# hashicorp/consul

Hardware: NVIDIA B200
Metric: million node-ticks/sec (higher is better)
Workload: dtype u32

## Files before the change

__graft_entry__.py:

```python
from __future__ import annotations

import os
import subprocess
import sys

ROOT = os.path.dirname(os.path.abspath(__file__))
CSRC = os.path.join(ROOT, "consul_b200", "csrc")
LIBGSIM = os.path.join(ROOT, "consul_b200", "libgsim.so")
LIBORACLE = os.path.join(ROOT, "oracle", "liboracle.so")
LIBHOSTEMU = os.path.join(ROOT, "tests", "hostemu", "libgsim_hostemu.so")
FACADE_DEMO = os.path.join(ROOT, "tests", "hostemu", "serf_facade_check")

NVCC_FLAGS = ["-gencode", "arch=compute_100a,code=sm_100a", "-lineinfo", "-O3", "-std=c++17", "-fmad=false",
              "-Xcompiler", "-fPIC", "-Xcompiler", "-ffp-contract=off", "-Xcompiler", "-pthread", "-shared"]


def _newer(target: str, sources) -> bool:
    if not os.path.exists(target):
        return False
    t = os.path.getmtime(target)
    return all(os.path.getmtime(s) <= t for s in sources)


def _run(cmd):
    print("+", " ".join(cmd), flush=True)
    subprocess.run(cmd, check=True, cwd=ROOT)


def _sources(*dirs_and_ext):
    out = []
    for d, exts in dirs_and_ext:
        for f in sorted(os.listdir(d)):
            if f.endswith(exts):
                out.append(os.path.join(d, f))
    return out


def build_oracle(force: bool = False) -> None:
    hdr = _sources((os.path.join(ROOT, "include"), (".h",)))
    osrc = [os.path.join(ROOT, "oracle", "oracle.cpp")]
    if force or not _newer(LIBORACLE, osrc + hdr):
        _run(["g++", "-O3", "-mavx2", "-ffp-contract=off", "-std=c++17", "-fopenmp", "-fPIC", "-shared", "-o",
              LIBORACLE] + osrc)


def build(force: bool = False) -> None:
    hdr = _sources((CSRC, (".h",)), (os.path.join(ROOT, "include"), (".h", ".hpp")))
    srcs = [os.path.join(CSRC, "gs_cuda.cu"), os.path.join(CSRC, "gs_vmm.cu"), os.path.join(CSRC, "gs_api.cpp")]
    if force or not _newer(LIBGSIM, srcs + hdr):
        nvcc = os.environ.get("NVCC", "nvcc")
        _run([nvcc] + NVCC_FLAGS + ["-o", LIBGSIM] + srcs)
    build_oracle(force)
    hsrc = [os.path.join(CSRC, "gs_api.cpp"), os.path.join(ROOT, "tests", "hostemu", "hostemu_backend.cpp")]
    if force or not _newer(LIBHOSTEMU, hsrc + hdr):
        _run(["g++", "-O2", "-ffp-contract=off", "-std=c++17", "-pthread", "-fPIC", "-shared",
              "-DGS_MAKE_BACKEND=gs_make_hostemu_backend", "-o", LIBHOSTEMU] + hsrc)
    sys.path.insert(0, ROOT)
    import consul_b200


def smoke() -> None:
    sys.path.insert(0, ROOT)
    sys.path.insert(0, os.path.join(ROOT, "tests"))
    if not (os.path.exists(LIBGSIM) and os.path.exists(LIBORACLE)):
        build()
    from consul_b200 import Pool, lan_config, PRED_ALL_RUMORS_CONVERGED
    from oracle_binding import OraclePool

    n = 4096
    cfg = lan_config(capacity=n + 1, n_initial=n, seed=0x5EED0001)
    gpu = Pool(cfg)
    ora = OraclePool(cfg)
    for p in (gpu, ora):
        x = p.member_add()
        assert p.join(x, [0]) == 1
    tg = gpu.run_until(PRED_ALL_RUMORS_CONVERGED, 0, 400, 1)
    to = ora.run_until(PRED_ALL_RUMORS_CONVERGED, 0, 400, 1)
    gpu.step(64)
    ora.step(64)
    hg, ho = gpu.state_hash(), ora.state_hash()
    assert tg == to, (tg, to)
    assert hg == ho, (hg, ho)
    assert gpu.launch_count() > 0
    print(f"smoke ok: n={n + 1} converged at tick {tg}, state hash {hg[0]:016x} == oracle, "
          f"{gpu.launch_count()} kernel launches")


if __name__ == "__main__":
    build(force="--force" in sys.argv)
    if "--smoke" in sys.argv:
        smoke()
```

consul_b200/csrc/gs_api.cpp:

```cpp
#include <math.h>
#include <stdio.h>
#include <stdlib.h>
#include <string.h>

#include <algorithm>
#include <mutex>
#include <string>
#include <type_traits>
#include <atomic>
#include <condition_variable>
#include <functional>
#include <thread>
#include <vector>

#include "../../include/gsim.h"
#include "gs_backend.h"
#include "gs_wire.h"
#include "gs_coord.h"

#ifndef GS_MAKE_BACKEND
#define GS_MAKE_BACKEND gs_make_cuda_backend
#endif
GsBackend* GS_MAKE_BACKEND(int device, char* err, size_t err_cap);

// ... 608 lines not shown
    okk = okk && acol(&tx16, GS_MAX_RUMORS / 2);
    d.tx = reinterpret_cast<uint8_t*>(tx16);
  }
  if (cfg->flags & GSIM_FLAG_COORDINATES) {
    if (sharded) {
      g_create_err = "network coordinates are not supported on sharded pools yet";
      fprintf(stderr, "libgsim: %s\n", g_create_err.c_str());
      gsim_pool_destroy(p);
      return GSIM_ERR_INVALID;
    }
    okk = okk && alloc_col(p, &d.coord, cap * 2 * GS_COORD_WORDS) && alloc_col(p, &d.ctag, cap * 2) &&
          alloc_col(p, &d.adj, cap * GS_ADJ_WINDOW) && alloc_col(p, &d.adj_idx, cap);
  }
  if (cfg->flags & GSIM_FLAG_PUSH_PULL)
    okk = okk && acol(&d.ppreq, 2 * GS_PPK) && acol(&d.pp_clk, 4);
  uint32_t evcap = cfg->event_log_capacity ? cfg->event_log_capacity : 65536u;
  if (!sharded) {
    okk = okk && alloc_col(p, &d.stats, (size_t)GSIM_STAT_COUNT);
    okk = okk && alloc_col(p, &d.heard_cnt, (size_t)32) && alloc_col(p, &d.conv_tick, (size_t)32);
    okk = okk && alloc_col(p, &d.view_cnt, (size_t)4);
    okk = okk && alloc_col(p, &d.crashed_alive, (size_t)1) && alloc_col(p, &d.crashed_dead_tick, (size_t)1);
    okk = okk && alloc_col(p, &d.evlog, (size_t)evcap) && alloc_col(p, &d.evlog_cursor, (size_t)2);
    okk = okk && alloc_col(p, &d.tick_base, (size_t)1);
    okk = okk && alloc_col(p, &d.done_ctr, (size_t)1);
    okk = okk && alloc_col(p, &d.qstate[0], (size_t)GS_Q_WORDS);
    okk = okk && alloc_col(p, &p->g_dev, (size_t)1);
  } else if (okk) {
    p->pages = reinterpret_cast<uint8_t*>(be->shard_alloc(GS_PAGE_BYTES, 1));
    okk = p->pages != nullptr && be->shard_commit(&p->shard_fds, &p->n_shard_fds);
    if (okk) {
      uint8_t* page0 = p->pages;
      uint8_t* mine = p->pages + (size_t)p->rank * GS_PAGE_BYTES;
      d.stats = reinterpret_cast<unsigned long long*>(mine + GS_PG_STATS);
      d.heard_cnt = reinterpret_cast<uint32_t*>(page0 + GS_PG_HEARD_CNT);
      d.conv_tick = reinterpret_cast<uint32_t*>(page0 + GS_PG_CONV_TICK);
      d.view_cnt = reinterpret_cast<uint32_t*>(page0 + GS_PG_VIEW_CNT);
      d.crashed_alive = reinterpret_cast<uint32_t*>(page0 + GS_PG_CRASHED_ALIVE);
      d.crashed_dead_tick = reinterpret_cast<uint32_t*>(page0 + GS_PG_CRASHED_DEAD_TICK);
      d.evlog_cursor = reinterpret_cast<uint32_t*>(page0 + GS_PG_EVLOG_CURSOR);
      d.evlog = reinterpret_cast<GsEventRec*>(page0 + GS_PG_EVLOG);
      const uint32_t room = (GS_PAGE_BYTES - GS_PG_EVLOG) / (uint32_t)sizeof(GsEventRec);
      if (evcap > room) evcap = room;
      d.tick_base = reinterpret_cast<uint32_t*>(mine + GS_PG_TICK_BASE);
      p->g_dev = reinterpret_cast<GsGlobals*>(mine + GS_PG_GLOBALS);
      for (uint32_t r = 0; r < GS_MAX_WORLD; ++r)
        p->xb.flags[r] = reinterpret_cast<uint32_t*>(p->pages + (size_t)(r < p->world ? r : 0) * GS_PAGE_BYTES + GS_PG_XBAR_FLAGS);
      for (uint32_t r = 0; r < GS_MAX_WORLD; ++r)
        d.tick_flags[r] = reinterpret_cast<uint32_t*>(p->pages + (size_t)(r < p->world ? r : 0) * GS_PAGE_BYTES + GS_PG_TICK_FLAGS);
      d.done_ctr = reinterpret_cast<uint32_t*>(mine + GS_PG_DONE_CTR);
      for (uint32_t r = 0; r < p->world; ++r)
        d.qstate[r] = reinterpret_cast<uint32_t*>(p->pages + (size_t)r * GS_PAGE_BYTES + GS_PG_QSTATE);
      p->xb.epoch = reinterpret_cast<uint32_t*>(mine + GS_PG_XBAR_EPOCH);
      p->xb.rank = p->rank;
      p->xb.world = p->world;
      okk = be->fill8(mine, 0, GS_PAGE_BYTES) && be->sync();
    }
  }
  if (!okk) {
    g_create_err = be->last_error();
    fprintf(stderr, "libgsim: allocation failed: %s\n", be->last_error());
    gsim_pool_destroy(p);
    return GSIM_ERR_NOMEM;
  }

  g.n = cfg->n_initial;
  p->n_established = cfg->n_initial;
  g.cap = (uint32_t)cap;
  g.up_count = cfg->n_initial;
  g.P = (uint32_t)(cfg->probe_interval_ns / tick);
  g.T = (uint32_t)(cfg->probe_timeout_ns / tick);
  g.GI = (uint32_t)(cfg->gossip_interval_ns / tick);
  g.gossip_nodes = cfg->gossip_nodes;
  g.indirect_checks = cfg->indirect_checks;
  g.awareness_max = cfg->awareness_max_multiplier;
  g.gtd_ticks = ceil_ticks(cfg->gossip_to_the_dead_ns, tick);
  g.udp_avail = cfg->udp_buffer_size > 2 ? cfg->udp_buffer_size - 2 : 0;
  g.disable_tcp = cfg->disable_tcp_pings;
  g.loss_thr = (uint32_t)(((uint64_t)cfg->packet_loss_ppm << 32) / 1000000ull);
  if (cfg->packet_loss_ppm >= 1000000u) g.loss_thr = 0xFFFFFFFFu;
  g.event_buffer = cfg->event_buffer;
  g.seed_lo = (uint32_t)cfg->seed;
  g.seed_hi = (uint32_t)(cfg->seed >> 32);
  g.flags = cfg->flags;
  g.evlog_cap = evcap;
  g.world = cfg->world_size;
  g.rank = cfg->rank;
  g.phase_group = phase_group;
  g.phase_gate = (phase_group % GS_TILE == 0) ? 1u : 0u;
  g.phase_shift = 0;
  while (g.phase_gate && (GS_TILE << g.phase_shift) < phase_group) g.phase_shift++;
  {
    const uint32_t rot = gs_phase_rot(g.seed_lo, g.seed_hi);
    g.rot_p = rot % g.P;
    g.rot_g = (rot >> 16) % g.GI;
  }
  g.rows_per_rank = (uint32_t)p->rows_per_rank;
  g.tick_seconds = (double)tick / 1.0e9;
  g.coord_base_rtt_s = 0.0005;
  recompute_tables(p);
  if (!sharded && init_device_state(p) != GSIM_OK) {
    g_create_err = be->last_error();
    fprintf(stderr, "libgsim: pool init failed: %s\n", be->last_error());
    gsim_pool_destroy(p);
    return GSIM_ERR_CUDA;
  }
  *out = p;
  return GSIM_OK;
}

extern "C" int gsim_shard_export_fds(gsim_pool* p, int* fds, size_t cap, size_t* n) {
  if (!p || !n || !p->sharded) return GSIM_ERR_INVALID;
  *n = p->n_shard_fds;
  if (fds) {
    if (cap < p->n_shard_fds) return GSIM_ERR_INVALID;
    memcpy(fds, p->shard_fds, p->n_shard_fds * sizeof(int));
  }
  return GSIM_OK;
}

extern "C" int gsim_shard_attach(gsim_pool* p, uint32_t peer_rank, const int* fds, size_t n) {
  if (!p || !p->sharded || p->ready || !fds) return GSIM_ERR_INVALID;
  std::lock_guard<std::mutex> lk(p->mu);
  if (!p->be->shard_attach(peer_rank, fds, n)) return fail(p, GSIM_ERR_CUDA, "shard_attach");
  p->attached += 1;
  return GSIM_OK;
}

extern "C" int gsim_shard_ready(gsim_pool* p) {
  if (!p) return GSIM_ERR_INVALID;
  if (!p->sharded) return GSIM_OK;
  std::lock_guard<std::mutex> lk(p->mu);
  if (p->ready) return GSIM_OK;
  if (p->attached != p->world) return fail(p, GSIM_ERR_STATE, "not every peer rank has been attached");
  if (!p->be->xbar_host(p->xb)) return fail(p, GSIM_ERR_CUDA, "barrier");
  int rc = controller_call(p, nullptr, 0, [&]() -> int { return init_device_state(p); });
  if (rc) return fail(p, rc, "init");
  p->ready = true;
  return GSIM_OK;
}

extern "C" void gsim_pool_destroy(gsim_pool* p) {
  if (!p) return;
  if (p->be) {
    p->be->sync();
    if (p->stage) p->be->host_free(p->stage);
    delete p->workers;
    p->workers = nullptr;
    for (void* q : p->allocs) p->be->release(q);
    delete p->be;
  }
  delete p;
}

static void shard_rows(const gsim_pool* p, uint32_t* first, uint32_t* count) {
  const uint32_t n = p->g.n;
  *first = 0;
  *count = n;
  if (p->sharded) {
    const uint64_t f = (uint64_t)p->rank * p->rows_per_rank;
    *first = f < n ? (uint32_t)f : n;
    *count = *first + p->rows_per_rank < n ? (uint32_t)p->rows_per_rank : n - *first;
  }
}

static int collective_recount(gsim_pool* p) {
  if (!p->sharded || !p->ready) return GSIM_OK;
// ... 1584 lines not shown
```

consul_b200/csrc/gs_cuda.cu:

```cuda
#include <cuda_runtime.h>
#include <stdio.h>
#include <stdlib.h>
#include <string.h>

#include <map>

#include "gs_aux.h"
#include "gs_backend.h"
#include "gs_vmm.h"

#define GS_BLOCK 256
#define GS_GRAPH_TICKS 64
#define GS_WIN_GRAPH 8

namespace {

template <bool COORDS>
struct DevSinkT {
  static constexpr bool kCoords = COORDS;
  uint32_t* s_stat;
  uint32_t* s_heard;
  uint32_t* s_q;
  __device__ __forceinline__ void activity() { s_q[0] = 1u; }
  __device__ __forceinline__ void horizon(uint32_t h) { atomicMin(&s_q[1], h); }
// ... 17 lines not shown
      e.reserved = 0u;
      d.evlog[pos] = e;
    } else {
      atomicAdd_system(&d.evlog_cursor[1], 1u);
    }
  }
};
typedef DevSinkT<false> DevSink;

#ifndef GS_MIN_BLOCKS
#define GS_MIN_BLOCKS 4
#endif
#define GS_WARPS (GS_BLOCK / 32)
#define GS_ROUND 4

__device__ __forceinline__ uint32_t gs_smem_addr(const void* p) { return (uint32_t)__cvta_generic_to_shared(p); }
__device__ __forceinline__ void gs_mbar_init(uint64_t* bar, uint32_t arrivals) {
  asm volatile("mbarrier.init.shared::cta.b64 [%0], %1;" ::"r"(gs_smem_addr(bar)), "r"(arrivals) : "memory");
}
__device__ __forceinline__ void gs_mbar_expect_tx(uint64_t* bar, uint32_t bytes) {
  asm volatile("mbarrier.arrive.expect_tx.shared::cta.b64 _, [%0], %1;" ::"r"(gs_smem_addr(bar)), "r"(bytes) : "memory");
}
__device__ __forceinline__ void gs_bulk_g2s(void* smem_dst, const void* gsrc, uint32_t bytes, uint64_t* bar) {
  asm volatile("cp.async.bulk.shared::cluster.global.mbarrier::complete_tx::bytes [%0], [%1], %2, [%3];" ::"r"(
                   gs_smem_addr(smem_dst)),
               "l"(gsrc), "r"(bytes), "r"(gs_smem_addr(bar))
               : "memory");
}
__device__ __forceinline__ bool gs_mbar_wait(uint64_t* bar, uint32_t parity) {
  for (uint32_t spin = 0; spin < (1u << 24); ++spin) {
    uint32_t done;
    asm volatile(
        "{\n\t.reg .pred p;\n\t"
        "mbarrier.try_wait.parity.shared::cta.b64 p, [%1], %2;\n\t"
        "selp.u32 %0, 1, 0, p;\n\t}"
        : "=r"(done)
        : "r"(gs_smem_addr(bar)), "r"(parity)
        : "memory");
    if (done) return true;
  }
  return false;
}

__device__ __forceinline__ void gs_ranks_wait(const GsDev& d, const GsGlobals& g, uint32_t t) {
  if (threadIdx.x < g.world) {
    uint32_t v;
    do {
      asm volatile("ld.acquire.sys.global.u32 %0, [%1];" : "=r"(v) : "l"(d.tick_flags[g.rank] + threadIdx.x) : "memory");
    } while ((int32_t)(v - t) < 0);
  }
  __syncthreads();
}
__device__ __forceinline__ void gs_ranks_release(const GsDev& d, const GsGlobals& g, uint32_t t_done) {
  __syncthreads();
  if (threadIdx.x == 0u) {
    __threadfence_system();
    const uint32_t arrived = atomicAdd(d.done_ctr, 1u);
    if (arrived == gridDim.x - 1u) {
      __threadfence_system();
      *d.done_ctr = 0u;
      __threadfence_system();
      for (uint32_t r = 0; r < g.world; ++r)
        asm volatile("st.release.sys.global.u32 [%0], %1;" ::"l"(d.tick_flags[r] + g.rank), "r"(t_done) : "memory");
    }
  }
}

__device__ __forceinline__ void gs_q_publish(const GsDev& d, const GsGlobals& g, const uint32_t* s_q, uint32_t t) {
  if (s_q[0] != 0u) {
    if (g.world <= 1u) atomicMax(d.qstate[0] + GS_Q_LAST_ACTIVE, t + 1u);
    else for (uint32_t r = 0; r < g.world; ++r) atomicMax_system(d.qstate[r] + GS_Q_LAST_ACTIVE, t + 1u);
  }
  if (s_q[1] != GS_NEVER) {
    if (g.world <= 1u) atomicMin(d.qstate[0] + GS_Q_HORIZON, s_q[1]);
    else for (uint32_t r = 0; r < g.world; ++r) atomicMin_system(d.qstate[r] + GS_Q_HORIZON, s_q[1]);
  }
}

template <bool COORDS>
__device__ __noinline__ void gs_row_step_call(const GsDev* dp, const GsGlobals* gp, uint32_t i, uint32_t t,
                                              uint32_t inb, uint32_t* s_stat, uint32_t* s_heard, uint32_t* s_q) {
  DevSinkT<COORDS> sink{s_stat, s_heard, s_q};
  gs_row_step(*dp, *gp, i, t, t % gp->GI, inb, sink);
}

template <bool COORDS>
__global__ void __launch_bounds__(GS_BLOCK, GS_MIN_BLOCKS)
    gs_tick_kernel(const __grid_constant__ GsDev d, const GsGlobals* __restrict__ gp, uint32_t k_off) {
  __shared__ uint32_t s_stat[GS_NSTAT * 32];
  __shared__ uint32_t s_heard[32 * 32];
  __shared__ __align__(128) uint32_t s_inb[GS_WARPS][GS_ROUND][GS_TILE];
  __shared__ __align__(128) uint32_t s_due[GS_WARPS][GS_ROUND][GS_TILE];
  __shared__ __align__(8) uint64_t s_bar[GS_WARPS];
  __shared__ uint32_t s_q[2];
  __shared__ uint32_t s_work[GS_WARPS * GS_ROUND * 4];
  __shared__ uint32_t s_wn[2], s_wtake[2];
  const uint32_t tid = threadIdx.x;
  for (uint32_t x = tid; x < GS_NSTAT * 32u; x += GS_BLOCK) s_stat[x] = 0u;
  for (uint32_t x = tid; x < 32u * 32u; x += GS_BLOCK) s_heard[x] = 0u;
  if (tid == 64u) s_q[0] = 0u;
  if (tid == 65u) s_q[1] = GS_NEVER;
  if (tid >= 66u && tid < 68u) s_wn[tid - 66u] = 0u;
  if (tid >= 68u && tid < 70u) s_wtake[tid - 68u] = 0u;
  if (tid >= 96u && tid < 96u + GS_WARPS) gs_mbar_init(&s_bar[tid - 96u], 1u);
  asm volatile("fence.mbarrier_init.release.cluster;" ::: "memory");
  asm volatile("griddepcontrol.launch_dependents;" ::: "memory");
  asm volatile("griddepcontrol.wait;" ::: "memory");
  __syncthreads();
  const GsGlobals& g = *gp;
  const uint32_t t = *d.tick_base + k_off;
  if (g.world > 1u) gs_ranks_wait(d, g, t);
  const uint32_t cur = t & 1u, P = g.P, pslot = t % P, gslot = t % g.GI;
  const uint32_t pslot_t = (t + P - g.T % P) % P;
  const uint32_t lane = tid & 31u, wib = tid >> 5;
  uint32_t tile_lo = 0, tile_hi = (g.n + GS_TILE - 1u) / GS_TILE;
  if (g.world > 1u) {
    const uint32_t per = g.rows_per_rank / GS_TILE;
    tile_lo = g.rank * per < tile_hi ? g.rank * per : tile_hi;
    tile_hi = tile_lo + per < tile_hi ? tile_lo + per : tile_hi;
  }
  const uint32_t n_warps = gridDim.x * GS_WARPS, n_tiles = tile_hi - tile_lo;
  const uint32_t wid = blockIdx.x * GS_WARPS + wib;
  const uint32_t t_begin = tile_lo + (uint32_t)(((uint64_t)wid * n_tiles) / n_warps);
  const uint32_t t_end = tile_lo + (uint32_t)(((uint64_t)(wid + 1u) * n_tiles) / n_warps);
  const uint32_t* __restrict__ inbox_cur = d.inbox[t & g.ring_mask];
  const bool gated = g.phase_gate != 0u;
  const uint32_t shift = g.phase_shift;
  DevSinkT<COORDS> sink{s_stat, s_heard, s_q};

  const uint32_t max_run = (n_tiles + n_warps - 1u) / n_warps, n_rounds = (max_run + GS_ROUND - 1u) / GS_ROUND;
  bool did_work = false;
  const bool sys_scan = g.world > 1u && (g.flags & 4u);
  auto bring = [&](uint32_t r) {
    const uint32_t b0 = t_begin + r * GS_ROUND < t_end ? t_begin + r * GS_ROUND : t_end;
    const uint32_t b1 = b0 + GS_ROUND < t_end ? b0 + GS_ROUND : t_end;
    const uint32_t tiles = b1 - b0;
    if (!tiles) return;
    uint32_t gate_mask = 0;
    for (uint32_t x = 0; x < tiles; ++x) {
      bool gate = true;
      if (gated) {
        const uint32_t pp = gs_probe_phase(g.rot_p, (b0 + x) >> shift, P);
        gate = pp == pslot || pp == pslot_t;
      }
      gate_mask |= gate ? 1u << x : 0u;
    }
    const size_t off0 = (size_t)b0 * GS_TILE;
    if (sys_scan) {
      for (uint32_t x = 0; x < tiles; ++x) {
        uint4 v;
        asm volatile("ld.relaxed.sys.global.v4.u32 {%0,%1,%2,%3}, [%4];"
                     : "=r"(v.x), "=r"(v.y), "=r"(v.z), "=r"(v.w) : "l"(inbox_cur + off0 + x * GS_TILE + lane * 4u) : "memory");
        *reinterpret_cast<uint4*>(&s_inb[wib][x][lane * 4u]) = v;
        const uint4 dv = (gate_mask >> x) & 1u ? *reinterpret_cast<const uint4*>(d.due + off0 + x * GS_TILE + lane * 4u)
                                               : make_uint4(GS_NEVER, GS_NEVER, GS_NEVER, GS_NEVER);
        *reinterpret_cast<uint4*>(&s_due[wib][x][lane * 4u]) = dv;
      }
      __syncwarp();
      return;
    }
    for (uint32_t x = 0; x < tiles; ++x)
      if (!((gate_mask >> x) & 1u))
        *reinterpret_cast<uint4*>(&s_due[wib][x][lane * 4u]) = make_uint4(GS_NEVER, GS_NEVER, GS_NEVER, GS_NEVER);
    __syncwarp();
    if (lane == 0u) {
      asm volatile("fence.proxy.async.shared::cta;" ::: "memory");
// ... 4 lines not shown
    }
  };
  bring(0u);
  for (uint32_t round = 0; round < n_rounds; ++round) {
  const uint32_t par = round & 1u;
  const uint32_t r_begin = t_begin + round * GS_ROUND < t_end ? t_begin + round * GS_ROUND : t_end;
  const uint32_t r_end = r_begin + GS_ROUND < t_end ? r_begin + GS_ROUND : t_end;
  if (r_end > r_begin && !sys_scan && !gs_mbar_wait(&s_bar[wib], round & 1u)) {
    if (lane == 0u) atomicExch(d.qstate[g.rank] + GS_Q_VIOLATION, t + 1u);
  }
  for (uint32_t tile = r_begin; tile < r_end; ++tile) {
    const uint32_t st = tile - r_begin;
    const uint4 i4 = *reinterpret_cast<const uint4*>(&s_inb[wib][st][lane * 4u]);
    const uint4 d4 = *reinterpret_cast<const uint4*>(&s_due[wib][st][lane * 4u]);
    bool mine = (i4.x | i4.y | i4.z | i4.w) != 0u || d4.x == t || d4.y == t || d4.z == t || d4.w == t;
    bool pp_tile = false;
    if (g.pp_interval != 0u) {
      if (gated) {
        pp_tile = gs_pp_due(g.pp_interval, g.rot_pp, tile >> shift, t);
      } else {
#pragma unroll
        for (uint32_t u = 0; u < 4u; ++u)
          pp_tile |= gs_pp_due(g.pp_interval, g.rot_pp, (tile * GS_TILE + lane * 4u + u) / g.phase_group, t);
      }
      mine |= pp_tile;
    }
    if (__any_sync(0xFFFFFFFFu, mine)) {
      did_work = true;
      __syncwarp();
      const uint32_t base = tile * GS_TILE + lane;
      bool act[4], cand[4];
      bool any_cand = false;
#pragma unroll
      for (int u = 0; u < 4; ++u) {
        const uint32_t w = s_inb[wib][st][u * 32 + lane];
        const bool due_now = s_due[wib][st][u * 32 + lane] == t;
        act[u] = w != 0u || due_now ||
                 (g.pp_interval != 0u && gs_pp_due(g.pp_interval, g.rot_pp, (base + 32u * u) / g.phase_group, t));
        cand[u] = w == 0u && due_now;
        any_cand |= cand[u];
      }
      if (__any_sync(0xFFFFFFFFu, any_cand)) {
        GsFastProbe f[4];
#pragma unroll
        for (int u = 0; u < 4; ++u)
          if (cand[u]) gs_fast_load(d, cur, base + 32u * u, f[u]);
#pragma unroll
        for (int u = 0; u < 4; ++u)
          if (cand[u]) cand[u] = gs_fast_target(d, g, cur, base + 32u * u, f[u]);
        uint32_t n_probe = 0, n_ack = 0;
#pragma unroll
        for (int u = 0; u < 4; ++u) {
          bool acked = false;
          const bool done = cand[u] && gs_fast_finish(d, g, sink, base + 32u * u, t, f[u], &acked);
          if (done) act[u] = false;
          n_probe += __popc(__ballot_sync(0xFFFFFFFFu, done));
          n_ack += __popc(__ballot_sync(0xFFFFFFFFu, done && acked));
        }
        if (lane == 0u && n_probe) {
          atomicAdd(&s_stat[GS_ST_PROBES * 32], n_probe);
          atomicAdd(&s_stat[GS_ST_ACTIVE_ROWS * 32], n_probe);
          if (n_ack) atomicAdd(&s_stat[GS_ST_ACKS * 32], n_ack);
        }
      }
#pragma unroll
      for (int u = 0; u < 4; ++u) {
        if (__any_sync(0xFFFFFFFFu, act[u]) && lane == 0u) s_work[atomicAdd(&s_wn[par], 1u)] = tile * 4u + (uint32_t)u;
      }
    }
  }
  __syncwarp();
  if (round + 1u < n_rounds) bring(round + 1u);
  __syncthreads();
  if (tid == 0u) s_wn[par ^ 1u] = s_wtake[par ^ 1u] = 0u;
  const uint32_t n_work = s_wn[par];
  for (;;) {
    uint32_t idx = 0;
    if (lane == 0u) idx = atomicAdd(&s_wtake[par], 1u);
    idx = __shfl_sync(0xFFFFFFFFu, idx, 0);
    if (idx >= n_work) break;
    did_work = true;
    const uint32_t i = s_work[idx] * 32u + lane;
    const uint32_t w = __ldcg(inbox_cur + i);
    const bool a = w != 0u || __ldcg(d.due + i) == t ||
                   (g.pp_interval != 0u && gs_pp_due(g.pp_interval, g.rot_pp, i / g.phase_group, t));
    if (a) gs_row_step_call<COORDS>(&d, gp, i, t, w, s_stat, s_heard, s_q);
  }
  __syncthreads();
  }
  if (g.world > 1u && did_work && !(g.flags & 8u)) __threadfence_system();
  __syncthreads();
  if (tid < GS_NSTAT) {
    uint32_t v = 0;
    for (uint32_t x = 0; x < 32u; ++x) v += s_stat[tid * 32u + ((x + tid) & 31u)];
    if (v) atomicAdd(&d.stats[tid], (unsigned long long)v);
  } else if (tid >= 32u && tid < 32u + GS_MAX_RUMORS) {
    uint32_t r = tid - 32u, c = 0;
    for (uint32_t x = 0; x < 32u; ++x) c += s_heard[r * 32u + ((x + r) & 31u)];
    if (c) {
      uint32_t old = atomicAdd_system(&d.heard_cnt[r], c);
      if (old + c == g.up_count) d.conv_tick[r] = t;
    }
  }
  if (tid == 0u) gs_q_publish(d, g, s_q, t);
  if (g.world > 1u) gs_ranks_release(d, g, t + 1u);
}

template <bool COORDS>
__device__ __noinline__ void gs_window_generic(const GsDev* dp, const GsGlobals* gp, uint32_t gb, uint32_t g_end,
                                               uint32_t tf00, uint32_t tf01, uint32_t tf02, uint32_t tf03,
                                               uint32_t tx00, uint32_t tx01, uint32_t tx02, uint32_t tx03,
                                               uint32_t t0, uint32_t w1, uint32_t* s_stat, uint32_t* s_heard,
                                               uint32_t* s_q, uint32_t* counts) {
  const GsDev& d = *dp;
  const GsGlobals& g = *gp;
  const GsHot h = gs_hot(g);
  const uint32_t P = h.P, T = h.T, lane = threadIdx.x & 31u;
  const uint32_t tf0[4] = {tf00, tf01, tf02, tf03}, tx0[4] = {tx00, tx01, tx02, tx03};
  const bool fast_ok = h.loss_thr == 0u && h.graph_n == 0u && d.coord == nullptr && h.pp_interval == 0u;
  DevSinkT<COORDS> sink{s_stat, s_heard, s_q};
  uint32_t n_probe = 0, n_ack = 0;
  bool did_work = false;
  (void)did_work;
#pragma unroll 1
    for (uint32_t s0 = t0; s0 < w1; s0 += P) {
    const uint32_t off = s0 - t0;
    uint32_t tf[4], tx[4], due[4];
    bool cand[4], slow[4];
    bool any_slow = false;
#pragma unroll
    for (int u = 0; u < 4; ++u) {
      if (gb + u < g_end) {
        tf[u] = tf0[u] + off;
        tx[u] = tx0[u] + off;
        due[u] = __ldcg(d.due + (gb + u) * 32u + lane);
      } else {
        tf[u] = tx[u] = GS_NEVER;
        due[u] = GS_NEVER - 1u;
      }
      cand[u] = fast_ok && due[u] == tf[u] && tf[u] < w1;
      slow[u] = (due[u] == tf[u] && tf[u] < w1 && !fast_ok) || (due[u] == tx[u] && tx[u] < w1);
    }
    GsFastProbe f[4];
#pragma unroll
    for (int u = 0; u < 4; ++u)
      if (cand[u]) gs_fast_load(d, tf[u] & 1u, (gb + u) * 32u + lane, f[u]);
#pragma unroll
    for (int u = 0; u < 4; ++u)
      if (cand[u]) {
        const bool okk = gs_fast_target(d, h, tf[u] & 1u, (gb + u) * 32u + lane, f[u]);
        if (!okk) { cand[u] = false; slow[u] = true; }
      }
#pragma unroll
    for (int u = 0; u < 4; ++u) {
      bool acked = false, done = false;
      if (cand[u]) {
        done = gs_fast_finish(d, h, sink, (gb + u) * 32u + lane, tf[u], f[u], &acked);
        if (!done) slow[u] = true;
        else if (!acked && tf[u] + T < w1) slow[u] = true;
      }
      n_probe += done ? 1u : 0u;
      n_ack += done && acked ? 1u : 0u;
      any_slow |= slow[u];
    }
    if (__any_sync(0xFFFFFFFFu, any_slow)) {
      did_work = true;
#pragma unroll 1
      for (int u = 0; u < 4; ++u) {
        const bool sl = u == 0 ? slow[0] : u == 1 ? slow[1] : u == 2 ? slow[2] : slow[3];
// ... 950 lines not shown
```

consul_b200/csrc/gs_row.h:

```cpp
#pragma once
#include <string.h>

#include "gs_core.h"
#include "gs_coord.h"

#if defined(__CUDA_ARCH__)
#define GS_DEV __device__ __forceinline__
__device__ __forceinline__ uint32_t gs_atomic_or_sys(uint32_t* p, uint32_t v) {
  uint32_t old;
  asm volatile("atom.global.sys.or.b32 %0, [%1], %2;" : "=r"(old) : "l"(p), "r"(v) : "memory");
  return old;
}
__device__ __forceinline__ uint64_t gs_atomic_min_sys(uint64_t* p, uint64_t v) {
  unsigned long long old;
  asm volatile("atom.global.sys.min.u64 %0, [%1], %2;" : "=l"(old) : "l"(p), "l"((unsigned long long)v) : "memory");
  return old;
}
__device__ __forceinline__ void gs_red_or_sys(uint32_t* p, uint32_t v) {
  asm volatile("red.global.sys.or.b32 [%0], %1;" ::"l"(p), "r"(v) : "memory");
}
#define GS_ATOMIC_OR32(p, v) (g.world > 1u ? gs_atomic_or_sys((p), (v)) : atomicOr((p), (v)))
#define GS_POST_OR32(p, v)                                                         \
  do {                                                                             \
    if (g.world <= 1u) (void)atomicOr((p), (v));                                   \
// ... 653 lines not shown
        }
      }
      for (uint32_t q = 0; q < np && queued != 0u; ++q) {
        uint32_t pkt = gs_select_packet(d, g, i, queued);
        if (pkt == 0u) break;
        uint32_t pm = pkt;
        while (pm) {
#if defined(__CUDA_ARCH__)
          uint32_t r = __ffs(pm) - 1;
#else
          uint32_t r = (uint32_t)__builtin_ctz(pm);
#endif
          pm &= pm - 1;
          uint32_t tx = (uint32_t)d.tx[GS_TX(r, cap, i)] + 1u;
          d.tx[GS_TX(r, cap, i)] = (uint8_t)tx;
          if (tx >= g.retransmit_limit) queued &= ~(1u << r);
          sink.stat(GS_ST_RUMORS_SENT, 1);
        }
        sink.stat(GS_ST_GOSSIP_PACKETS, 1);
        if (!gs_lost(g, sink, i, peers[q], t, GS_LK_GOSSIP, q))
          gs_post(d, g, sink, (t + 1u + gs_extra(g, i, peers[q])) & g.ring_mask, peers[q], pkt);
      }
      if (queued != q0) d.queued[i] = queued;
    }

    if (pp_now && !(m & GS_META_ISOLATED)) {
      uint32_t partner[1];
      if (gs_krandom(d, g, i, t, GS_PUR_PUSHPULL, 1u, 1u, GS_EMPTY32, m, partner) != 0u) {
        const uint32_t j = partner[0];
        uint32_t* req = d.ppreq + (size_t)nxt * GS_PPK * cap;
        uint32_t v = i;
        for (uint32_t s = 0; s < GS_PPK; ++s) {
          const uint32_t old = GS_ATOMIC_MIN32(&req[(size_t)s * cap + j], v);
          if (old == v || old == GS_EMPTY32) break;
          if (old > v) v = old;
        }
        uint32_t* clk = d.pp_clk + (size_t)nxt * 2u * cap;
        GS_ATOMIC_MAX32(&clk[j], d.ltime_member[i]);
        GS_ATOMIC_MAX32(&clk[cap + j], d.ltime_event[i]);
        gs_post(d, g, sink, inxt, j, (d.heard[i] & g.active_mask) | GS_ACC_BIT);
        sink.stat(GS_ST_PUSH_PULLS, 1);
      }
    }
  }

  if (k != k0) {
    gs_key_store(d, g, nxt, i, k);
    m |= GS_META_DIRTY;
  } else if (m0 & GS_META_DIRTY) {
    gs_key_store(d, g, nxt, i, k);
    m &= ~GS_META_DIRTY;
  }
  if (m != m0) d.meta[i] = m;
  if (due != due0) d.due[i] = due;
  if (gs_key_rank(k) == GS_RANK_SUSPECT || (m & GS_META_DIRTY) || queued != 0u)
    gs_post(d, g, sink, inxt, i, GS_WAKE_BIT);
}

struct GsFastProbe {
  uint32_t k, m, cursor, pass, c, kc;
};

GS_DEV void gs_fast_load(const GsDev& d, uint32_t cur, uint32_t i, GsFastProbe& f) {
  f.k = d.key[cur][i];
  f.m = d.meta[i];
  f.cursor = d.cursor[i];
  f.pass = d.pass[i];
}

template <class G>
GS_DEV bool gs_fast_target(const GsDev& d, const G& g, uint32_t cur, uint32_t i,
                           GsFastProbe& f) {
  if (g.loss_thr != 0u || g.graph_n != 0u || d.coord != nullptr) return false;
  if (gs_key_truth(f.k) != GS_TRUTH_UP || gs_key_rank(f.k) != GS_RANK_ALIVE) return false;
  if (gs_meta_stage(f.m) != GS_STAGE_IDLE || (f.m & (GS_META_DIRTY | GS_META_ISOLATED))) return false;
  if (f.cursor >= g.n) return false;
  GsU4 rk = gs_perm_keys(g.seed_lo, g.seed_hi, i, f.pass);
  f.c = gs_perm(f.cursor, g.n, g.perm_bits, rk);
  if (f.c == i) return false;
  f.kc = gs_peer_key(d, cur, f.c, false);
  return true;
}

template <class G, class Sink>
GS_DEV bool gs_fast_finish(const GsDev& d, const G& g, Sink& sink, uint32_t i, uint32_t t,
                           const GsFastProbe& f, bool* acked) {
  const uint32_t rank = gs_key_rank(f.kc);
  if (gs_key_truth(f.kc) == GS_TRUTH_NONE || rank == GS_RANK_DEAD || rank == GS_RANK_LEFT ||
      gs_key_pending(f.kc))
    return false;
  if (g.pp_interval != 0u && gs_pp_due(g.pp_interval, g.rot_pp, i / g.phase_group, t))
    return false;
  uint32_t m = f.m;
  if (gs_key_truth(f.kc) == GS_TRUTH_UP && gs_extra(g, i, f.c) + gs_extra(g, f.c, i) <= g.T) {
    const uint32_t aw = gs_meta_aw(m);
    m = gs_meta_set_aw(m, aw ? aw - 1u : 0u);
    d.due[i] = t + g.P;
    *acked = true;
  } else {
    m = gs_meta_set_stage(m, GS_STAGE_WAIT_T);
    d.probe_tgt[i] = f.c;
    d.probe_inc[i] = GS_PEER_INC(d, t & 1u, f.c, f.kc);
    d.due[i] = t + g.T;
    sink.horizon(t + g.P);
    *acked = false;
  }
  d.cursor[i] = f.cursor + 1u;
  if (m != f.m) d.meta[i] = m;
  return true;
}
```

consul_b200/pool.py:

```python
from __future__ import annotations

import ctypes as C
from dataclasses import dataclass

import numpy as np

from . import _lib
from ._lib import (COLUMNS, GSIM_MAX_RUMORS, GSIM_MAX_SUSPICION_SLOTS, STAT_NAMES, GsimConfig,
                   GsimEvent, GsimMember, GsimMemberDesc, GsimRumorInfo, GsimStats)

PRED_RUMOR_CONVERGED = 1
PRED_ALL_RUMORS_CONVERGED = 2
PRED_CRASHED_ALL_DEAD = 3
NEVER = 0xFFFFFFFF

FLAG_LOG_GLOBAL_EVENTS = 1
FLAG_NO_GRAPH = 2
FLAG_NO_WINDOWS = 16
FLAG_PUSH_PULL = 32
FLAG_COORDINATES = 64
MEMBER_WATCHED = 1


class GsimError(RuntimeError):
    def __init__(self, code: int, msg: str):
        super().__init__(f"gsim error {code}: {msg}")
        self.code = code


def lan_config(lib=None, **kw) -> GsimConfig:
    lib = lib or _lib.lib()
    c = GsimConfig()
    lib.gsim_config_default_lan(C.byref(c))
    for k, v in kw.items():
        setattr(c, k, v)
    return c


def wan_config(lib=None, **kw) -> GsimConfig:
    lib = lib or _lib.lib()
    c = GsimConfig()
    lib.gsim_config_default_wan(C.byref(c))
    for k, v in kw.items():
        setattr(c, k, v)
    return c


def consul_test_config(lib=None, **kw) -> GsimConfig:
    lib = lib or _lib.lib()
    c = GsimConfig()
    lib.gsim_config_consul_test(C.byref(c))
    for k, v in kw.items():
        setattr(c, k, v)
    return c


@dataclass
class Event:
    tick: int
    type: int
    subject: int
    observer: int
    ltime: int


class Pool:
    def __init__(self, cfg: GsimConfig, lib=None):
        self.lib = lib or _lib.lib()
        self.cfg = cfg
        h = C.c_void_p()
        rc = self.lib.gsim_pool_create(C.byref(cfg), C.byref(h))
        if rc != 0:
            raise GsimError(rc, self.lib.gsim_strerror(rc).decode())
        self.h = h
        self.capacity = cfg.capacity

    def close(self):
        if getattr(self, "h", None):
            self.lib.gsim_pool_destroy(self.h)
            self.h = None

    def __del__(self):
        try:
            self.close()
        except Exception:
            pass

    def __enter__(self):
        return self

    def __exit__(self, *a):
        self.close()

    def _ck(self, rc: int):
        if rc != 0:
            msg = self.lib.gsim_last_error(self.h).decode() or self.lib.gsim_strerror(rc).decode()
            raise GsimError(rc, msg)

    def member_add(self, alive_msg_size: int = 0, watched: bool = False, name_len: int = 0, meta_len: int = 0) -> int:
        d = GsimMemberDesc(alive_msg_size, MEMBER_WATCHED if watched else 0, name_len, meta_len)
        out = C.c_uint32()
        self._ck(self.lib.gsim_member_add(self.h, C.byref(d), C.byref(out)))
        return out.value
# ... 172 lines not shown
```

include/gsim.h:

```cpp
#ifndef GSIM_H
#define GSIM_H

#include <stddef.h>
#include <stdint.h>

#ifdef __cplusplus
extern "C" {
#endif

#define GSIM_ABI_VERSION 1

#define GSIM_OK 0
#define GSIM_ERR_INVALID (-1)
#define GSIM_ERR_NO_DEVICE (-2)
#define GSIM_ERR_CUDA (-3)
#define GSIM_ERR_CAPACITY (-4)
#define GSIM_ERR_NOT_FOUND (-5)
#define GSIM_ERR_STATE (-6)
#define GSIM_ERR_TOO_LARGE (-7)
#define GSIM_ERR_NOMEM (-8)

#define GSIM_STATUS_NONE 0
#define GSIM_STATUS_ALIVE 1
#define GSIM_STATUS_LEAVING 2
#define GSIM_STATUS_LEFT 3
#define GSIM_STATUS_FAILED 4
#define GSIM_STATUS_REAP (-1)

#define GSIM_RANK_ALIVE 0
#define GSIM_RANK_SUSPECT 1
#define GSIM_RANK_DEAD 2
#define GSIM_RANK_LEFT 3

#define GSIM_TRUTH_NONE 0
#define GSIM_TRUTH_UP 1
#define GSIM_TRUTH_CRASHED 2
#define GSIM_TRUTH_GONE 3

#define GSIM_EVENT_MEMBER_JOIN 0
#define GSIM_EVENT_MEMBER_LEAVE 1
#define GSIM_EVENT_MEMBER_FAILED 2
#define GSIM_EVENT_MEMBER_UPDATE 3
#define GSIM_EVENT_MEMBER_REAP 4
#define GSIM_EVENT_USER 5
#define GSIM_EVENT_QUERY 6

#define GSIM_RUMOR_FREE 0
#define GSIM_RUMOR_ALIVE 1
#define GSIM_RUMOR_JOIN_INTENT 2
#define GSIM_RUMOR_LEAVE_INTENT 3
#define GSIM_RUMOR_USER_EVENT 4
#define GSIM_RUMOR_UPDATE 5
#define GSIM_MAX_RUMORS 30
#define GSIM_MAX_SUSPICION_SLOTS 5

typedef struct gsim_pool gsim_pool;

typedef struct gsim_config {
  uint32_t struct_size;
  uint32_t flags;
  uint64_t seed;
  uint32_t capacity;
  uint32_t n_initial;
  uint64_t tick_ns;
  uint64_t probe_interval_ns;
  uint64_t probe_timeout_ns;
  uint64_t gossip_interval_ns;
  uint64_t gossip_to_the_dead_ns;
  uint64_t push_pull_interval_ns;
  uint32_t gossip_nodes;
  uint32_t indirect_checks;
  uint32_t retransmit_mult;
  uint32_t suspicion_mult;
  uint32_t suspicion_max_timeout_mult;
  uint32_t awareness_max_multiplier;
  uint32_t udp_buffer_size;
  uint32_t disable_tcp_pings;
  uint32_t packet_loss_ppm;
  uint32_t event_buffer;
  uint32_t user_event_size_limit;
  uint64_t leave_propagate_delay_ns;
  uint64_t broadcast_timeout_ns;
  uint64_t reap_interval_ns;
  uint64_t reconnect_timeout_ns;
  uint64_t tombstone_timeout_ns;
  uint32_t world_size;
  uint32_t rank;
  int32_t device;
  uint32_t event_log_capacity;
  uint32_t phase_group;
  uint32_t mailbox_depth;
} gsim_config;

#define GSIM_FLAG_LOG_GLOBAL_EVENTS 1u
#define GSIM_FLAG_NO_GRAPH 2u
#define GSIM_FLAG_SHARD_SYNC_SCAN 4u
#define GSIM_FLAG_SHARD_LEAN_FENCE 8u
#define GSIM_FLAG_NO_WINDOWS 16u
#define GSIM_FLAG_PUSH_PULL 32u
#define GSIM_FLAG_SHARD_ATOM 128u
#define GSIM_FLAG_COORDINATES 64u

void gsim_config_default_lan(gsim_config* cfg);
void gsim_config_default_wan(gsim_config* cfg);
void gsim_config_consul_test(gsim_config* cfg);

uint32_t gsim_retransmit_limit(uint32_t retransmit_mult, uint32_t n);
uint64_t gsim_suspicion_timeout_ns(uint32_t suspicion_mult, uint32_t n, uint64_t interval_ns);
int64_t gsim_remaining_suspicion_ns(uint32_t n_confirm, uint32_t k, uint64_t elapsed_ns,
                                    uint64_t min_ns, uint64_t max_ns);
uint64_t gsim_push_pull_scale_ns(uint64_t interval_ns, uint32_t n);
uint32_t gsim_lamport_witness(uint32_t clock, uint32_t v);
uint32_t gsim_refute_incarnation(uint32_t cur, uint32_t accused);
void gsim_philox4x32(const uint32_t ctr[4], const uint32_t key[2], uint32_t out[4]);

int gsim_pool_create(const gsim_config* cfg, gsim_pool** out);
void gsim_pool_destroy(gsim_pool* p);
const char* gsim_strerror(int code);
const char* gsim_last_error(gsim_pool* p);
int gsim_abi_version(void);

typedef struct gsim_member_desc {
  uint32_t alive_msg_size;
  uint32_t flags;
  uint32_t name_len;
  uint32_t meta_len;
} gsim_member_desc;
#define GSIM_MEMBER_WATCHED 1u

int gsim_member_add(gsim_pool* p, const gsim_member_desc* desc, uint32_t* id_out);

int gsim_join(gsim_pool* p, uint32_t id, const uint32_t* seeds, size_t n_seeds, int ignore_old,
              int* n_ok);
int gsim_leave(gsim_pool* p, uint32_t id);
int gsim_crash(gsim_pool* p, uint32_t id);
int gsim_crash_many(gsim_pool* p, const uint32_t* ids, size_t n);
int gsim_crash_fraction(gsim_pool* p, uint32_t ppm, uint32_t salt, uint32_t* n_crashed);
int gsim_force_leave(gsim_pool* p, uint32_t via, uint32_t target, int prune);
int gsim_user_event(gsim_pool* p, uint32_t id, const void* name, size_t name_len,
                    const void* payload, size_t payload_len, int coalesce, uint32_t* slot_out);

int gsim_rumor_inject(gsim_pool* p, uint32_t slot, uint32_t id, int* accepted);

int gsim_member_update(gsim_pool* p, uint32_t id, uint32_t alive_msg_size, uint32_t* slot_out);

int gsim_graph_set(gsim_pool* p, uint32_t n_rows, const uint32_t* row_ptr, const uint32_t* col_idx);

int gsim_member_reconnect_timeout_set(gsim_pool* p, uint32_t id, uint64_t timeout_ns);

int gsim_coordinate_get(gsim_pool* p, uint32_t id, double out[11]);

int gsim_member_watch(gsim_pool* p, uint32_t id, int on);

int gsim_latency_set(gsim_pool* p, uint32_t n_dcs, const uint8_t* lat_ticks);

int gsim_step(gsim_pool* p, uint32_t ticks);
#define GSIM_PRED_RUMOR_CONVERGED 1
#define GSIM_PRED_ALL_RUMORS_CONVERGED 2
#define GSIM_PRED_CRASHED_ALL_DEAD 3
int gsim_run_until(gsim_pool* p, int predicate, uint32_t arg, uint32_t max_ticks,
                   uint32_t check_every, uint32_t* tick_out);
uint32_t gsim_now(gsim_pool* p);

typedef struct gsim_member {
  uint32_t id;
  int32_t status;
  uint32_t incarnation;
  uint32_t rank;
} gsim_member;
int gsim_members(gsim_pool* p, uint32_t observer, gsim_member* out, size_t cap, size_t* n);
int gsim_num_nodes(gsim_pool* p, uint32_t observer, uint32_t* n);

typedef struct gsim_event {
  uint32_t tick;
  uint32_t type;
  uint32_t subject;
  uint32_t observer;
  uint32_t ltime;
  uint32_t reserved;
} gsim_event;
int gsim_poll_events(gsim_pool* p, gsim_event* out, size_t cap, size_t* n);

typedef struct gsim_rumor_info {
  uint32_t kind, subject, incarnation, ltime, origin, size_bytes, start_tick;
// ... 101 lines not shown
```

Baseline: 568,600.

## Add fast-path gossip handler for common inbox rows bypassing full row step

Adds a specialized device path, gs_fast_gossip, that handles rows receiving simple alive/intent rumors and doing a routine gossip round and probe. It reads only the needed columns, packs transmit counters for up to four rumor pairs, and posts gossip packets directly. The full gs_row_step runs only when the fast path rejects the row. This targets the cost of the general per-row state machine on the hot gossip path, in exchange for duplicated logic that must stay bit-identical with the oracle, plus an extra noinline call for every row with inbox traffic.

New measurement: 670,700, median of 6. 17.9% higher.

```diff
diff --git a/__graft_entry__.py b/__graft_entry__.py
--- a/__graft_entry__.py
+++ b/__graft_entry__.py
@@ -51,8 +51,9 @@
         nvcc = os.environ.get("NVCC", "nvcc")
         _run([nvcc] + NVCC_FLAGS + ["-o", LIBGSIM] + srcs)
     build_oracle(force)
-    hsrc = [os.path.join(CSRC, "gs_api.cpp"), os.path.join(ROOT, "tests", "hostemu", "hostemu_backend.cpp")]
-    if force or not _newer(LIBHOSTEMU, hsrc + hdr):
+    hsrc = [os.path.join(CSRC, "gs_api.cpp"), os.path.join(ROOT, "tests", "hostemu", "hostemu_tiers.cpp")]
+    hdeps = [os.path.join(ROOT, "tests", "hostemu", "hostemu_backend.cpp")]
+    if force or not _newer(LIBHOSTEMU, hsrc + hdeps + hdr):
         _run(["g++", "-O2", "-ffp-contract=off", "-std=c++17", "-pthread", "-fPIC", "-shared",
               "-DGS_MAKE_BACKEND=gs_make_hostemu_backend", "-o", LIBHOSTEMU] + hsrc)
     sys.path.insert(0, ROOT)
diff --git a/consul_b200/csrc/gs_api.cpp b/consul_b200/csrc/gs_api.cpp
--- a/consul_b200/csrc/gs_api.cpp
+++ b/consul_b200/csrc/gs_api.cpp
@@ -714,6 +714,7 @@
   g.seed_lo = (uint32_t)cfg->seed;
   g.seed_hi = (uint32_t)(cfg->seed >> 32);
   g.flags = cfg->flags;
+  if (getenv("GSIM_NO_FAST_GOSSIP") != nullptr) g.flags |= GSIM_FLAG_NO_FAST_GOSSIP;
   g.evlog_cap = evcap;
   g.world = cfg->world_size;
   g.rank = cfg->rank;
diff --git a/consul_b200/csrc/gs_cuda.cu b/consul_b200/csrc/gs_cuda.cu
--- a/consul_b200/csrc/gs_cuda.cu
+++ b/consul_b200/csrc/gs_cuda.cu
@@ -123,6 +123,14 @@
                                               uint32_t inb, uint32_t* s_stat, uint32_t* s_heard, uint32_t* s_q) {
   DevSinkT<COORDS> sink{s_stat, s_heard, s_q};
   gs_row_step(*dp, *gp, i, t, t % gp->GI, inb, sink);
+}
+
+template <bool COORDS>
+__device__ __noinline__ bool gs_fast_gossip_call(const GsDev* dp, const GsGlobals* gp, uint32_t i, uint32_t t,
+                                                 uint32_t gslot, uint32_t inb, bool due_now, uint32_t* s_stat,
+                                                 uint32_t* s_heard, uint32_t* s_q) {
+  DevSinkT<COORDS> sink{s_stat, s_heard, s_q};
+  return gs_fast_gossip(*dp, *gp, sink, i, t, gslot, inb, due_now);
 }
 
 template <bool COORDS>
@@ -293,9 +301,11 @@
     did_work = true;
     const uint32_t i = s_work[idx] * 32u + lane;
     const uint32_t w = __ldcg(inbox_cur + i);
-    const bool a = w != 0u || __ldcg(d.due + i) == t ||
+    const bool due_now = __ldcg(d.due + i) == t;
+    const bool a = w != 0u || due_now ||
                    (g.pp_interval != 0u && gs_pp_due(g.pp_interval, g.rot_pp, i / g.phase_group, t));
-    if (a) gs_row_step_call<COORDS>(&d, gp, i, t, w, s_stat, s_heard, s_q);
+    const bool fast = w != 0u && gs_fast_gossip_call<COORDS>(&d, gp, i, t, gslot, w, due_now, s_stat, s_heard, s_q);
+    if (a && !fast) gs_row_step_call<COORDS>(&d, gp, i, t, w, s_stat, s_heard, s_q);
   }
   __syncthreads();
   }
diff --git a/consul_b200/csrc/gs_row.h b/consul_b200/csrc/gs_row.h
--- a/consul_b200/csrc/gs_row.h
+++ b/consul_b200/csrc/gs_row.h
@@ -759,15 +759,21 @@
   return true;
 }
 
-template <class G, class Sink>
-GS_DEV bool gs_fast_finish(const GsDev& d, const G& g, Sink& sink, uint32_t i, uint32_t t,
-                           const GsFastProbe& f, bool* acked) {
+template <class G>
+GS_DEV bool gs_fast_accept(const G& g, uint32_t i, uint32_t t, const GsFastProbe& f) {
   const uint32_t rank = gs_key_rank(f.kc);
   if (gs_key_truth(f.kc) == GS_TRUTH_NONE || rank == GS_RANK_DEAD || rank == GS_RANK_LEFT ||
       gs_key_pending(f.kc))
     return false;
   if (g.pp_interval != 0u && gs_pp_due(g.pp_interval, g.rot_pp, i / g.phase_group, t))
     return false;
+  return true;
+}
+
+template <class G, class Sink>
+GS_DEV bool gs_fast_finish(const GsDev& d, const G& g, Sink& sink, uint32_t i, uint32_t t,
+                           const GsFastProbe& f, bool* acked) {
+  if (!gs_fast_accept(g, i, t, f)) return false;
   uint32_t m = f.m;
   if (gs_key_truth(f.kc) == GS_TRUTH_UP && gs_extra(g, i, f.c) + gs_extra(g, f.c, i) <= g.T) {
     const uint32_t aw = gs_meta_aw(m);
@@ -786,3 +792,161 @@
   if (m != f.m) d.meta[i] = m;
   return true;
 }
+
+#define GS_FG_PAIRS 4u
+
+GS_DEV uint32_t gs_popc(uint32_t x) {
+#if defined(__CUDA_ARCH__)
+  return __popc(x);
+#else
+  return (uint32_t)__builtin_popcount(x);
+#endif
+}
+GS_DEV uint32_t gs_lowbit(uint32_t x) {
+#if defined(__CUDA_ARCH__)
+  return __ffs(x) - 1;
+#else
+  return (uint32_t)__builtin_ctz(x);
+#endif
+}
+
+template <class Sink>
+GS_DEV bool gs_fast_gossip(const GsDev& d, const GsGlobals& g, Sink& sink, uint32_t i, uint32_t t, uint32_t gslot,
+                           uint32_t inb, bool due_now) {
+  const uint32_t am = g.active_mask;
+  uint32_t pm = 0;
+  for (uint32_t x = am; x != 0u; x &= x - 1u) pm |= 1u << (gs_lowbit(x) >> 1);
+  if (inb == 0u || (inb & GS_ACC_BIT) || (g.flags & 256u) || g.loss_thr != 0u || g.graph_n != 0u || g.n_dcs != 0u ||
+      g.pp_interval != 0u || g.active_bytes > g.udp_avail || g.n < 2u || g.gossip_nodes == 0u ||
+      gs_popc(pm) > GS_FG_PAIRS)
+    return false;
+  const uint32_t cur = t & 1u;
+  const size_t cap = g.cap;
+
+  GsFastProbe f;
+  f.k = d.key[cur][i];
+  f.m = d.meta[i];
+  const uint32_t q0 = d.queued[i], heard0 = d.heard[i];
+  const uint32_t rbits = inb & ~(GS_ACC_BIT | GS_WAKE_BIT) & am;
+  const uint32_t lt0 = rbits != 0u ? d.ltime_member[i] : 0u;
+  if (due_now) {
+    f.cursor = d.cursor[i];
+    f.pass = d.pass[i];
+  }
+  const uint32_t m0 = f.m;
+  if (gs_key_truth(f.k) != GS_TRUTH_UP || gs_key_rank(f.k) != GS_RANK_ALIVE ||
+      (m0 & (GS_META_DIRTY | GS_META_ISOLATED | GS_META_LEAVING)) || (q0 & ~am))
+    return false;
+  if (due_now && gs_meta_stage(m0) != GS_STAGE_IDLE) return false;
+  const uint32_t fresh = rbits & ~heard0;
+  uint32_t lt = lt0;
+  if (fresh != 0u) {
+    if (m0 & GS_META_WATCHED) return false;
+    for (uint32_t fm = fresh; fm != 0u; fm &= fm - 1u) {
+      const GsRumor& ru = g.rumors[gs_lowbit(fm)];
+      if (ru.kind == GS_RUMOR_JOIN_INTENT || ru.kind == GS_RUMOR_LEAVE_INTENT) {
+        if (ru.ltime >= lt) lt = ru.ltime + 1u;
+      } else if (ru.kind != GS_RUMOR_ALIVE) {
+        return false;
+      }
+    }
+  }
+  const uint32_t q1 = q0 | fresh;
+  const bool gossip = gslot == gs_meta_gphase(m0) && q1 != 0u;
+
+  if (due_now && !gs_fast_target(d, g, cur, i, f)) return false;
+  uint32_t cc[4], kc[4], txw[2] = {0u, 0u};
+  if (gossip) {
+    const GsU4 blk = gs_philox(g.seed_lo, g.seed_hi, i, t, GS_PUR_GOSSIP, 0u);
+#pragma unroll
+    for (uint32_t x = 0; x < 4u; ++x) {
+      cc[x] = gs_fastmod(gs_u4_get(blk, x), g.n, g.n_magic);
+      kc[x] = cc[x] != i ? gs_peer_key(d, cur, cc[x], false) : 0u;
+    }
+    uint32_t mm = pm;
+#pragma unroll
+    for (uint32_t x = 0; x < GS_FG_PAIRS; ++x) {
+      if (mm != 0u) {
+        const uint32_t p = gs_lowbit(mm);
+        mm &= mm - 1u;
+        const uint32_t w = *reinterpret_cast<const uint16_t*>(d.tx + GS_TX(2u * p, cap, i));
+        txw[x >> 1] |= w << ((x & 1u) * 16u);
+      }
+    }
+  }
+  if (due_now && !gs_fast_accept(g, i, t, f)) return false;
+  const uint32_t want = g.gossip_nodes > 8u ? 8u : g.gossip_nodes;
+  uint32_t np = 0, sel = 0;
+  if (gossip) {
+#pragma unroll
+    for (uint32_t x = 0; x < 4u; ++x) {
+      if (np < want) {
+        const uint32_t c = cc[x], k = kc[x], rank = gs_key_rank(k);
+        bool take = c != i && gs_key_truth(k) != GS_TRUTH_NONE && rank != GS_RANK_LEFT;
+        if (take && (rank == GS_RANK_DEAD || gs_key_pending(k))) return false;
+#pragma unroll
+        for (uint32_t y = 0; y < x; ++y) take = take && !(((sel >> y) & 1u) && cc[y] == c);
+        if (take) {
+          sel |= 1u << x;
+          ++np;
+        }
+      }
+    }
+    if (np < want) return false;
+  }
+
+  const uint32_t inxt = (t + 1u) & g.ring_mask;
+  sink.activity();
+  d.inbox[t & g.ring_mask][i] = 0u;
+  sink.stat(GS_ST_ACTIVE_ROWS, 1);
+  if (fresh != 0u) {
+    for (uint32_t fm = fresh; fm != 0u; fm &= fm - 1u) {
+      const uint32_t r = gs_lowbit(fm);
+      d.tx[GS_TX(r, cap, i)] = 0;
+      sink.heard(r);
+    }
+    sink.stat(GS_ST_RUMORS_ACCEPTED, gs_popc(fresh));
+    d.heard[i] = heard0 | fresh;
+    if (lt != lt0) d.ltime_member[i] = lt;
+  }
+  if (due_now) {
+    bool acked = false;
+    (void)gs_fast_finish(d, g, sink, i, t, f, &acked);
+    sink.stat(GS_ST_PROBES, 1);
+    if (acked) sink.stat(GS_ST_ACKS, 1);
+  }
+  uint32_t q = q1;
+  if (gossip) {
+    const uint32_t lim = g.retransmit_limit;
+    uint32_t pk0 = 0, pk1 = 0, pk2 = 0, pk3 = 0, n_pkts = 0, sent = 0;
+    for (uint32_t qm = q1; qm != 0u; qm &= qm - 1u) {
+      const uint32_t r = gs_lowbit(qm), x = gs_popc(pm & ((1u << (r >> 1)) - 1u));
+      const uint32_t tx = (fresh >> r) & 1u ? 0u : ((x >> 1 ? txw[1] : txw[0]) >> ((x & 1u) * 16u + (r & 1u) * 8u)) & 0xFFu;
+      const uint32_t room = lim > tx ? lim - tx : 1u;
+      const uint32_t s = room < np ? room : np;
+      d.tx[GS_TX(r, cap, i)] = (uint8_t)(tx + s);
+      if (tx + s >= lim) q &= ~(1u << r);
+      sent += s;
+      if (s > n_pkts) n_pkts = s;
+      pk0 |= 1u << r;
+      pk1 |= s > 1u ? 1u << r : 0u;
+      pk2 |= s > 2u ? 1u << r : 0u;
+      pk3 |= s > 3u ? 1u << r : 0u;
+    }
+    sink.stat(GS_ST_RUMORS_SENT, sent);
+    sink.stat(GS_ST_GOSSIP_PACKETS, n_pkts);
+#pragma unroll
+    for (uint32_t x = 0; x < 4u; ++x) {
+      if ((sel >> x) & 1u) {
+        if (pk0 != 0u) gs_post(d, g, sink, inxt, cc[x], pk0);
+        pk0 = pk1;
+        pk1 = pk2;
+        pk2 = pk3;
+        pk3 = 0u;
+      }
+    }
+  }
+  if (q != q0) d.queued[i] = q;
+  if (q != 0u) gs_post(d, g, sink, inxt, i, GS_WAKE_BIT);
+  return true;
+}
diff --git a/consul_b200/pool.py b/consul_b200/pool.py
--- a/consul_b200/pool.py
+++ b/consul_b200/pool.py
@@ -19,6 +19,7 @@
 FLAG_NO_WINDOWS = 16
 FLAG_PUSH_PULL = 32
 FLAG_COORDINATES = 64
+FLAG_NO_FAST_GOSSIP = 256
 MEMBER_WATCHED = 1
 
 
diff --git a/include/gsim.h b/include/gsim.h
--- a/include/gsim.h
+++ b/include/gsim.h
@@ -100,6 +100,7 @@
 #define GSIM_FLAG_PUSH_PULL 32u
 #define GSIM_FLAG_SHARD_ATOM 128u
 #define GSIM_FLAG_COORDINATES 64u
+#define GSIM_FLAG_NO_FAST_GOSSIP 256u
 
 void gsim_config_default_lan(gsim_config* cfg);
 void gsim_config_default_wan(gsim_config* cfg);
```
